# ashual/scene_generation

Measured on AMD Instinct MI355X. Metric: images/sec G+D step, 128x128 <=8-obj scene graphs, higher is better.
Workload: dtype f32

## Files before the change

scene_generation_amd/csrc/common.h:

```cpp
#pragma once
#include <hip/hip_runtime.h>
#include <stdint.h>
#include <stdio.h>
#include <atomic>
#include "../../include/sg2im_hip.h"

#define SG_WAVE 64

void sg_set_error(const char* fmt, ...);
int sg_check_indices_if_enabled(const int64_t* idx, int64_t n, int64_t lo, int64_t hi, const char* what, hipStream_t s);

#define SG_ARG_CHECK(cond, ...)                 \
  do {                                          \
    if (!(cond)) {                              \
      sg_set_error(__VA_ARGS__);                \
      return -1;                                \
    }                                           \
  } while (0)

#define SG_LAUNCH_CHECK(name)                                               \
  do {                                                                      \
    hipError_t e__ = hipGetLastError();                                     \
    if (e__ != hipSuccess) {                                                \
      sg_set_error("%s: launch failed: %s", name, hipGetErrorString(e__)); \
// ... 24 lines not shown
  SG_OPT_BN_BLOCKS,
  SG_OPT_INSTNORM_REG,
  SG_OPT_WGRAD_XCD,
  SG_OPT_WINO_REUSE,
  SG_OPT_WINO_FOLD_CELLS,
  SG_OPT_WINO_PIPE,
  SG_OPT_CHECK_INDICES,
  SG_OPT_LAST_BLOCK,
  SG_OPT_WINO_GEMM_TILE,
  SG_OPT_WINO43,
  SG_OPT_GCONV_FUSED_GATHER,
  SG_OPT_W24_GEMM_TILE,
  SG_OPT_WINO_IN_FUSE,
  SG_OPT_W43_NSUB,
  SG_OPT_W43_KFOLD,
  SG_OPT_WAVE_PRIO,
  SG_OPT_PAR_XCD_CHUNK,
  SG_OPT_W43_TAIL_SPLIT,
  SG_OPT_TAIL_SMAX,
  SG_OPT_TAIL_KTMIN,
  SG_OPT_W43_WGRAD_TILE,
  SG_OPT_PAR_SPLIT,
  SG_OPT_TAIL_CAPTURE,
  SG_OPT_COUNT
};
extern std::atomic<int> g_sg_opt[SG_OPT_COUNT];
static inline int sg_opt(int id) { return g_sg_opt[id].load(std::memory_order_relaxed); }
extern FILE* g_sg_launch_log;

enum {
  SG_K_IGEMM_BASE = 0, SG_K_IGEMM_COUNT = 48,
  SG_K_LINEAR = 48, SG_K_LAYOUT_FWD, SG_K_LAYOUT_BWD, SG_K_INSTNORM, SG_K_BATCHNORM, SG_K_ADAM, SG_K_SEGSUM,
  SG_K_CROP, SG_K_OTHER,
  SG_K_WINO_GEMM_128, SG_K_WINO_GEMM_64, SG_K_WINO_XFORM,
  SG_K_HEAD,
  SG_K_INSTNORM_BWD,
  SG_K_WINO24_GEMM,
  SG_K_WINO43_GEMM,
  SG_K_LAYOUT_TEST_PLANES,
  SG_K_DEPROCESS,
  SG_K_LAYOUT_RGB,
  SG_K_KMEANS_ASSIGN, SG_K_KMEANS_UPDATE, SG_K_KMEANS_RELOCATE, SG_K_KMEANS_PP,
  SG_K_SCENEGRAPH_CENTERS, SG_K_SCENEGRAPH_DERIVE, SG_K_SCENEGRAPH_AGREE,
  SG_K_MAXPOOL3S2, SG_K_ADD_RELU, SG_K_BN_FOLD, SG_K_SGD, SG_K_CLASSIFY_STATS,
  SG_K_RECT_CONV_T64, SG_K_RECT_CONV_T32, SG_K_RECT_CONV_T64W, SG_K_RECT_REDUCE, SG_K_INCEPTION_POOL, SG_K_RESIZE_BILINEAR,
  SG_K_SOFTMAX_ROWS, SG_K_INCEPTION_SCORE,
// ... 93 lines not shown
```

scene_generation_amd/csrc/igemm.hip:

```cpp
#include "igemm_core.h"

namespace sgk {
thread_local double t_alg_bytes = 0.0;
std::mutex g_tab_mu;
std::map<TabKey, TabEntry> g_tabs;
size_t g_tab_bytes = 0;
}

namespace {
int check_desc(const sgConvDesc* d, const char* who) {
  SG_ARG_CHECK(d != nullptr, "%s: null desc", who);
  SG_ARG_CHECK(d->KS == 1 || d->KS == 3 || d->KS == 4 || d->KS == 7, "%s: kernel size %d unsupported", who, d->KS);
  SG_ARG_CHECK(d->stride == 1 || d->stride == 2, "%s: stride %d unsupported", who, d->stride);
  SG_ARG_CHECK(d->upsample == 1 || d->upsample == 2, "%s: upsample %d unsupported", who, d->upsample);
  SG_ARG_CHECK(d->N > 0 && d->C1 > 0 && d->C2 >= 0 && d->Cout > 0 && d->H > 0 && d->W > 0 && d->OH > 0 && d->OW > 0,
               "%s: non-positive dimension", who);
  SG_ARG_CHECK(!d->pad_reflect || d->pad < d->H * d->upsample, "%s: reflect pad too large", who);
  const double lim = SG_MAX_ELEMS;
  SG_ARG_CHECK((double)d->N * (d->C1 + d->C2) * d->H * d->W <= lim && (double)d->N * d->Cout * d->OH * d->OW <= lim &&
                   (double)d->N * (d->C1 + d->C2) * (d->H * d->upsample + 2.0 * d->pad) *
                           (d->W * d->upsample + 2.0 * d->pad) <= lim &&
                   (double)d->Cout * (d->C1 + d->C2) * d->KS * d->KS <= lim,
               "%s: a tensor has more than %.0f elements (32-bit offsets%s)", who, lim,
               SG_BUFLOAD ? ", buffer-load range masking" : "");
// ... 119 lines not shown
extern "C" int sg_conv2d_wgrad(const sgConvDesc* d, const float* gy, const float* x1, const float* x2, float* gw,
                               float* gb, void* ws, size_t ws_bytes, sgStream stream) {
  if (check_desc(d, "sg_conv2d_wgrad")) return -1;
  sgk::t_alg_bytes = 4.0 * ((double)d->N * (d->C1 + d->C2) * d->H * d->W + (double)d->Cout * (d->C1 + d->C2) * d->KS * d->KS + (double)d->N * d->Cout * d->OH * d->OW);
  SG_ARG_CHECK(gy && x1 && gw, "sg_conv2d_wgrad: null pointer");
  SG_ARG_CHECK(d->C2 == 0 || x2, "sg_conv2d_wgrad: C2>0 but x2 null");
  hipStream_t s = (hipStream_t)stream;
  Gather g = make_gather(x1, x2, d->C1, d->C2, d->H, d->W, d->upsample, d->OH, d->OW, d->stride, d->pad, d->pad_reflect);
  g.bcast2 = d->x2_broadcast;
  const double flops = 2.0 * d->Cout * (double)(d->C1 + d->C2) * d->KS * d->KS * d->N * d->OH * d->OW;
  bool gb_done = false;
  if (int rc = sgk::nk_run(d->KS, gy, d->Cout, d->Cout, g, d->N, gw, ws, ws ? ws_bytes : 0, flops, s, nullptr, gb, &gb_done)) return rc;
  SG_LAUNCH_CHECK("sg_conv2d_wgrad");
  if (gb && !gb_done) return sg_channel_sum(gy, gb, d->N, d->Cout, d->OH * d->OW, ws, ws ? ws_bytes : 0, stream);
  return 0;
}


static int check_sparse(const sgConvDesc* d, const int32_t* list, const int32_t* cnt, int L, const char* who) {
  SG_ARG_CHECK(list && cnt, "%s: null channel list", who);
  SG_ARG_CHECK(L > 0 && L <= d->C1 + d->C2, "%s: L=%d outside (0, %d]", who, L, d->C1 + d->C2);
  return 0;
}
extern "C" size_t sg_conv2d_sparse_ws_bytes(const sgConvDesc* d, int L, int kind) {
  if (!d || L <= 0) return 0;
  const int KS2 = d->KS * d->KS;
  if (kind == 0) return sparse_fwd_ws(d->N, d->Cout, L, KS2);
  const size_t a = sparse_wgrad_ws(d->N, d->Cout, d->C1 + d->C2, L, KS2), cs = sg_channel_sum_ws_bytes(d->Cout);
  return a > cs ? a : cs;
}
extern "C" int sg_conv2d_fwd_sparse(const sgConvDesc* d, const float* x1, const float* x2, const float* w,
                                    const float* bias, const int32_t* chan_list, const int32_t* chan_cnt, int L, float* y,
                                    int act, float slope, void* ws, size_t ws_bytes, sgStream stream) {
  if (check_desc(d, "sg_conv2d_fwd_sparse") || check_sparse(d, chan_list, chan_cnt, L, "sg_conv2d_fwd_sparse")) return -1;
  sgk::t_alg_bytes = 4.0 * ((double)d->N * L * d->H * d->W + (double)d->N * d->Cout * L * d->KS * d->KS + (double)d->N * d->Cout * d->OH * d->OW);
  SG_ARG_CHECK(x1 && w && y && ws, "sg_conv2d_fwd_sparse: null pointer");
  SG_ARG_CHECK(d->C2 == 0 || x2, "sg_conv2d_fwd_sparse: C2>0 but x2 null");
  SG_ARG_CHECK(ws_bytes >= sg_conv2d_sparse_ws_bytes(d, L, 0), "sg_conv2d_fwd_sparse: workspace too small");
  hipStream_t s = (hipStream_t)stream;
  const int K = (d->C1 + d->C2) * d->KS * d->KS;
  Gather g = make_gather(x1, x2, d->C1, d->C2, d->H, d->W, d->upsample, d->OH, d->OW, d->stride, d->pad, d->pad_reflect);
  g.bcast2 = d->x2_broadcast;
  const Sparse sp{chan_list, chan_cnt, L, nullptr, nullptr};
  int rc = sgk::kn_sparse_run(d->KS, w, d->Cout, K, g, d->N, bias, y, act, slope, sp, ws, s);
  SG_LAUNCH_CHECK("sg_conv2d_fwd_sparse");
  return rc;
}
extern "C" int sg_conv2d_wgrad_sparse(const sgConvDesc* d, const float* gy, const float* x1, const float* x2,
                                      const int32_t* chan_list, const int32_t* chan_cnt, int L, float* gw, float* gb,
                                      void* ws, size_t ws_bytes, sgStream stream) {
  if (check_desc(d, "sg_conv2d_wgrad_sparse") || check_sparse(d, chan_list, chan_cnt, L, "sg_conv2d_wgrad_sparse")) return -1;
  sgk::t_alg_bytes = 4.0 * ((double)d->N * L * d->H * d->W + (double)d->N * d->Cout * L * d->KS * d->KS + (double)d->N * d->Cout * d->OH * d->OW);
  SG_ARG_CHECK(gy && x1 && gw && ws, "sg_conv2d_wgrad_sparse: null pointer");
  SG_ARG_CHECK(d->C2 == 0 || x2, "sg_conv2d_wgrad_sparse: C2>0 but x2 null");
  SG_ARG_CHECK(ws_bytes >= sg_conv2d_sparse_ws_bytes(d, L, 2), "sg_conv2d_wgrad_sparse: workspace too small");
  hipStream_t s = (hipStream_t)stream;
  Gather g = make_gather(x1, x2, d->C1, d->C2, d->H, d->W, d->upsample, d->OH, d->OW, d->stride, d->pad, d->pad_reflect);
  g.bcast2 = d->x2_broadcast;
  const Sparse sp{chan_list, chan_cnt, L, nullptr, nullptr};
  if (int rc = sgk::nk_run(d->KS, gy, d->Cout, d->Cout, g, d->N, gw, ws, ws_bytes, 0.0, s, &sp)) return rc;
  SG_LAUNCH_CHECK("sg_conv2d_wgrad_sparse");
  if (gb) return sg_channel_sum(gy, gb, d->N, d->Cout, d->OH * d->OW, ws, ws_bytes, stream);
  return 0;
}
extern "C" int sg_conv2d_fwd_perimage(const sgConvDesc* d, const float* x1, const float* x2, const float* wimg,
                                      const float* bias, const int32_t* chan_list, const int32_t* chan_cnt, int L, float* y,
                                      int act, float slope, void* ws, size_t ws_bytes, sgStream stream) {
  if (check_desc(d, "sg_conv2d_fwd_perimage") || check_sparse(d, chan_list, chan_cnt, L, "sg_conv2d_fwd_perimage")) return -1;
  sgk::t_alg_bytes = 4.0 * ((double)d->N * L * d->H * d->W + (double)d->N * d->Cout * L * d->KS * d->KS + (double)d->N * d->Cout * d->OH * d->OW);
  SG_ARG_CHECK(x1 && wimg && y && ws, "sg_conv2d_fwd_perimage: null pointer");
  SG_ARG_CHECK(d->C2 == 0 || x2, "sg_conv2d_fwd_perimage: C2>0 but x2 null");
  SG_ARG_CHECK(ws_bytes >= sg_conv2d_sparse_ws_bytes(d, L, 0), "sg_conv2d_fwd_perimage: workspace too small");
  hipStream_t s = (hipStream_t)stream;
  const int K = (d->C1 + d->C2) * d->KS * d->KS;
  Gather g = make_gather(x1, x2, d->C1, d->C2, d->H, d->W, d->upsample, d->OH, d->OW, d->stride, d->pad, d->pad_reflect);
  g.bcast2 = d->x2_broadcast;
  const Sparse sp{chan_list, chan_cnt, L, wimg, nullptr};
  int rc = sgk::kn_sparse_run(d->KS, nullptr, d->Cout, K, g, d->N, bias, y, act, slope, sp, ws, s);
  SG_LAUNCH_CHECK("sg_conv2d_fwd_perimage");
  return rc;
}
extern "C" int sg_conv2d_wgrad_perimage(const sgConvDesc* d, const float* gy, const float* x1, const float* x2,
                                        const int32_t* chan_list, const int32_t* chan_cnt, int L, float* gwimg, void* ws,
                                        size_t ws_bytes, sgStream stream) {
  if (check_desc(d, "sg_conv2d_wgrad_perimage") || check_sparse(d, chan_list, chan_cnt, L, "sg_conv2d_wgrad_perimage")) return -1;
  sgk::t_alg_bytes = 4.0 * ((double)d->N * L * d->H * d->W + (double)d->N * d->Cout * L * d->KS * d->KS + (double)d->N * d->Cout * d->OH * d->OW);
  SG_ARG_CHECK(gy && x1 && gwimg && ws, "sg_conv2d_wgrad_perimage: null pointer");
  SG_ARG_CHECK(d->C2 == 0 || x2, "sg_conv2d_wgrad_perimage: C2>0 but x2 null");
  SG_ARG_CHECK(ws_bytes >= sg_conv2d_sparse_ws_bytes(d, L, 2), "sg_conv2d_wgrad_perimage: workspace too small");
  hipStream_t s = (hipStream_t)stream;
  Gather g = make_gather(x1, x2, d->C1, d->C2, d->H, d->W, d->upsample, d->OH, d->OW, d->stride, d->pad, d->pad_reflect);
  g.bcast2 = d->x2_broadcast;
  const Sparse sp{chan_list, chan_cnt, L, nullptr, gwimg};
  if (int rc = sgk::nk_run(d->KS, gy, d->Cout, d->Cout, g, d->N, nullptr, ws, ws_bytes, 0.0, s, &sp)) return rc;
  SG_LAUNCH_CHECK("sg_conv2d_wgrad_perimage");
  return 0;
}

extern "C" int sg_convT2d_fwd(const sgConvDesc* d, const float* x, const float* w, const float* bias, float* y,
                              void* ws, size_t ws_bytes, sgStream stream) {
  if (check_desc(d, "sg_convT2d_fwd")) return -1;
  sgk::t_alg_bytes = 4.0 * ((double)d->N * (d->C1) * d->H * d->W + (double)d->Cout * (d->C1) * d->KS * d->KS + (double)d->N * d->Cout * d->OH * d->OW);
  SG_ARG_CHECK(x && w && y && ws, "sg_convT2d_fwd: null pointer");
  const int Cin = d->C1, R = d->KS * d->KS;
  SG_ARG_CHECK(d->C2 == 0 && d->upsample == 1 && !d->pad_reflect, "sg_convT2d_fwd: unsupported desc");
  SG_ARG_CHECK(ws_bytes >= (size_t)d->Cout * Cin * R * sizeof(float) + ktab_bytes(Cin * R),
               "sg_convT2d_fwd: workspace too small");
  hipStream_t s = (hipStream_t)stream;
  const TgArgs ta = tg_args(d, SG_TG_CONVT_FWD, 0, 0);
  Gather g = make_gather(x, nullptr, Cin, 0, d->H, d->W, 1, ta.PH, ta.PW, d->stride, ta.pad, 0);
  const double flops = 2.0 * d->Cout * Cin * R * (double)d->N * d->H * d->W;
  if (ta.parity) {
    SG_ARG_CHECK(ws_bytes >= parity_ws(d->Cout, Cin, R), "sg_convT2d_fwd: workspace too small");
    int rc = sgk::kn_parity_run(d->KS, w, Cin, d->Cout, 0, ta.M, g, d->N, bias, y, d->Cout, SG_ACT_NONE, 0.f, flops, ws,
                              ws_bytes, s);
    SG_LAUNCH_CHECK("sg_convT2d_fwd");
// ... 2130 lines not shown
```

scene_generation_amd/csrc/igemm_core.h:

```cpp
#pragma once
#include <type_traits>
#include "common.h"
#include <stdlib.h>
#include <array>
#include <map>
#include <mutex>

typedef float f32x16 __attribute__((ext_vector_type(16)));


namespace sgk {
struct Gather {
  const float* src1; const float* src2;
  int C1, C2;
  int SH, SW;
  int LH, LW;
  int ushift;
  int PH, PW;
  int stride, sshift, pad, reflect;
  int bcast2;
  int pstep, ph0, pw0;
};

struct KEntry { unsigned choff; unsigned tapsel; };
struct Sparse { const int* list; const int* cnt; int L; const float* wimg; float* gwimg; };
struct TabEntry { void* dev; size_t bytes; hipEvent_t ready; hipStream_t stream; };
using TabKey = std::array<long long, 12>;
extern thread_local double t_alg_bytes;
extern std::mutex g_tab_mu;
extern std::map<TabKey, TabEntry> g_tabs;
extern size_t g_tab_bytes;

int kn0_run(int KS, const float* A, int M, int K, const Gather& g, int NB, const float* bias, float* out, int Mtot, int act,
            float slope, double flops, void* ktab_ws, size_t ws_avail, hipStream_t s);
int kn1_run(int KS, const float* A, int M, int K, const Gather& g, int NB, const float* bias, float* out, int Mtot, int act,
            float slope, double flops, void* ktab_ws, size_t ws_avail, unsigned variant_stride, hipStream_t s);
int kn_sparse_run(int KS, const float* W, int M, int K, const Gather& g, int NB, const float* bias, float* out, int act,
                  float slope, const Sparse& sp, void* ws, hipStream_t s);
int kn_parity_run(int KS, const float* W, int Rdim, int B, int m0, int M, const Gather& g, int NB, const float* bias,
                  float* out, int Mtot, int act, float slope, double flops, void* ws, size_t ws_bytes, hipStream_t s);
int nk_run(int KS, const float* A, int M, int Mtot, const Gather& g, int NB, float* out, void* ws, size_t ws_bytes,
           double flops, hipStream_t s, const Sparse* sp, float* gb = nullptr, bool* gb_done = nullptr);
int skinny_vec(int align, int ld, int K);
int skinny_gemm(const float* a, int lda, int av, const float* b, int ldb, int bv, float* c, const float* bias,
                float* rowsum, int M, int N, int K, int act, float slope, hipStream_t s);
int skinny_gemm_gather(const float* obj, const float* pred, const int64_t* edges, int T, int Do, int Dp, const float* w, float* c,
                       const float* bias, int N, int act, float slope, hipStream_t s);
inline bool skinny_shape(int M, int N) {
// ... 730 lines not shown
#endif
    const bool ok = !MASK || o1 >= 0;
    const unsigned b1 = ok ? (unsigned)o1 : 0u;
    const unsigned b2 = (TWO && ok) ? (unsigned)buf[2 * KBLK + kl_] : 0u;
#pragma unroll
    for (int j = 0; j < COLS; ++j) {
      if (TWO) {
        const bool second = (secmask_ >> j) & 1u;
        const float* base = second ? g.src2 : g.src1;
        st.r[j] = base[(second ? b2 : b1) + choff_[j]];
      } else {
        st.r[j] = g.src1[b1 + choff_[j]];
      }
    }
    st.ok = ok ? 1u : 0u;
  }
  __device__ __forceinline__ void store(const Stage& st, float* T) const {
    const bool ok = !MASK || st.ok != 0u;
#pragma unroll
    for (int j = 0; j < COLS; ++j) T[(nr_ + 16 * j) * LDK + kl_] = ok ? st.r[j] : 0.f;
  }
};

template <int ACT> __device__ __forceinline__ float act_fixed(float v, int act, float slope) {
  if constexpr (ACT == SG_ACT_NONE) return v;
  else if constexpr (ACT == SG_ACT_RELU) return v > 0.f ? v : 0.f;
  else if constexpr (ACT == SG_ACT_LEAKY) return v > 0.f ? v : v * slope;
  else return sg_apply_act(v, act, slope);
}
template <int A> struct ActTag { static constexpr int value = A; };
template <class F> __device__ __forceinline__ void ep_dispatch(bool full, int act, F&& f) {
  if (full && act == SG_ACT_NONE) f(ActTag<SG_ACT_NONE>{});
  else if (full && act == SG_ACT_LEAKY) f(ActTag<SG_ACT_LEAKY>{});
  else if (full && act == SG_ACT_RELU) f(ActTag<SG_ACT_RELU>{});
  else f(ActTag<-1>{});
}

struct EpNCHW {
  float* out; const float* bias; int PHW, Mtot, M, Npix, act; float slope; size_t zstride;
  int PWs, step, h0, w0, PWf, PHWf;
  FastDiv dPHW, dPWs;
  __device__ __forceinline__ void set_limit(int n) { Npix = n; }
  template <int TM, int TN>
  __device__ __forceinline__ void store(f32x16 (&acc)[TM][TN], int mbase, int nbase, int lane, int z) const {
    const bool full = mbase + 32 * TM <= M && nbase + 32 * TN <= Npix;
    const int mrow = mbase + 4 * (lane >> 5);
// ... 963 lines not shown
  } else {
    t.Rdim = d->Cout; t.M = c_end - c_begin; t.PH = d->H; t.PW = d->W; t.pad = 1;
  }
  t.K = t.Rdim * R;
  t.a_off = t.parity ? 0 : (entry == SG_TG_CONVT_FWD ? 0 : (size_t)c_begin * t.K);
  t.ws_off = t.parity ? 0 : nw * sizeof(float);
  if (entry == SG_TG_DGRAD_FOLDED) {
    const size_t VS = (size_t)d->N * d->Cout * d->OH * d->OW;
    t.variants = (unsigned)VS;
    t.ws_off = (((nw + 63) / 64) * 64 + 9 * VS) * sizeof(float);
  }
  return t;
}

inline int sparse_kc(int L, int KS2) { return sg_cdiv(L * KS2, BK) * BK; }
inline int sparse_kpad(int L, int KS2) { return sg_cdiv(sparse_kc(L, KS2), 64) * 64 + 128; }
inline size_t sparse_fwd_ws(int NB, int M, int L, int KS2) {
  return (size_t)NB * ((size_t)sparse_kpad(L, KS2) * sizeof(KEntry) + (size_t)M * sparse_kc(L, KS2) * sizeof(float) + 64);
}
inline size_t parity_ws(int M, int Rdim, int KS2) { return (size_t)M * Rdim * KS2 * sizeof(float) + 64; }
inline size_t sparse_wgrad_ws(int NB, int M, int C, int L, int KS2) {
  return (size_t)NB * M * (sg_cdiv(L, 128) * 128) * KS2 * sizeof(float) + (size_t)NB * C * sizeof(int);
}
struct NkPlan { int tile; bool tap; int cpad; int splits; };
inline NkPlan nk_plan(int M, int C, int KS2, int Kpix, bool two) {
  NkPlan p;
  p.tap = C >= 48 || two;
  p.tile = M <= 32 ? 2 : 1;
  if (M > 64 && p.tap) {
    const double w128 = (double)sg_cdiv(M, 128) * 128 * sg_cdiv(C, 128) * 128;
    const double w64 = (double)sg_cdiv(M, 64) * 64 * sg_cdiv(C, 64) * 64;
    if (w128 * 0.7 < w64) p.tile = 0;
  }
  const int BMt = p.tile == 0 ? 128 : ((p.tile == 1 || p.tile == 3) ? 64 : 32), BNt = p.tile == 1 ? 64 : 128;
  p.cpad = p.tap ? sg_cdiv(C, BNt) * BNt : 0;
  const long tiles = (long)sg_cdiv(M, BMt) * (p.tap ? (long)KS2 * (p.cpad / BNt) : (long)sg_cdiv((long)C * KS2, BNt));
  const int target = p.tile == 0 ? 768 : 1024;
  int s = (int)((target + tiles - 1) / tiles);
  const int maxs = Kpix / (BK * 8) > 0 ? Kpix / (BK * 8) : 1;
  if (s > maxs) s = maxs;
  const int cap = p.tap ? 64 : 256;
  if (s > cap) s = cap;
  if (sg_opt(SG_OPT_WGRAD_XCD) && s >= 6) {
    int s8 = (s + 7) / 8 * 8;
    if (s8 > maxs) s8 = maxs / 8 * 8;
    if (s8 >= 8) s = s8;
// ... 7 lines not shown
```

scene_generation_amd/csrc/igemm_nk.hip:

```cpp
#include "igemm_core.h"

namespace {
__global__ void sparse_inv_kernel(const int* list, const int* cnt, int L, int C, int* inv) {
  const int b = blockIdx.y, c = blockIdx.x * blockDim.x + threadIdx.x;
  if (c >= C) return;
  int pos = -1;
  const int n = cnt[b];
  for (int j = 0; j < n; ++j) pos = list[b * L + j] == c ? j : pos;
  inv[b * C + c] = pos;
}
__global__ void sparse_wgrad_reduce_kernel(const float* slabs, const int* inv, float* gw, int M, int C, int KS2, int cpad,
                                           int NB) {
  const size_t i = (size_t)blockIdx.x * blockDim.x + threadIdx.x;
  if (i >= (size_t)M * C * KS2) return;
  const int t = (int)(i % KS2);
  const int c = (int)((i / KS2) % C);
  const int m = (int)(i / ((size_t)KS2 * C));
  float v = 0.f;
  for (int b = 0; b < NB; ++b) {
    const int j = inv[b * C + c];
    if (j >= 0) v += slabs[(((size_t)b * M + m) * KS2 + t) * cpad + j];
  }
  gw[i] = v;
}
// ... 9 lines not shown
                                             int NB) {
  const size_t i = (size_t)blockIdx.x * blockDim.x + threadIdx.x;
  if (i >= (size_t)NB * M * L * KS2) return;
  const int t = (int)(i % KS2);
  const int j = (int)((i / KS2) % L);
  const size_t bm = i / ((size_t)KS2 * L);
  const int b = (int)(bm / M);
  gwimg[i] = j < cnt[b] ? slabs[(bm * KS2 + t) * cpad + j] : 0.f;
}
__global__ void wgrad_unpermute_reduce_kernel(const float* __restrict__ slabs, float* __restrict__ gw, int M, int C, int KS2,
                                              int cpad, int S, const float* __restrict__ rowsum, float* __restrict__ gb) {
  const unsigned j = blockIdx.x * blockDim.x + threadIdx.x;
  const int m = blockIdx.y;
  if (gb && j == 0) {
    const float b = sg_sum_strided(rowsum + m, (size_t)M, S);
    gb[m] = b;
  }
  if (j >= (unsigned)(C * KS2)) return;
  const unsigned c = j / (unsigned)KS2, t = j - c * (unsigned)KS2;
  const size_t zs = (size_t)M * KS2 * cpad;
  const float* p = slabs + ((size_t)m * KS2 + t) * cpad + c;
  const float v = sg_sum_strided(p, zs, S);
  gw[(size_t)m * C * KS2 + j] = v;
}
template <int KS>
void launch_nk_general(int tile, const float* A, int M, int Mtot, int PQ, const Gather& g, int Ncols, const EpRowMajor& ep,
                       int Kpix, int splits, hipStream_t s, const Sparse* sp = nullptr, int zdiv = 1) {
  float* const rowsum = nullptr;
  const FastDiv dPQ((unsigned)PQ);
  const int* sl = sp ? sp->list : nullptr; const int* sc = sp ? sp->cnt : nullptr; const int L = sp ? sp->L : 0;
  if (tile == 2)
    launch_cfg<CfgW32>(LoadPixK<32>{A, M, Mtot, PQ, dPQ, rowsum}, LoadGatherNK<128, KS, false, true, NSW>{g, Ncols, sl, sc, L, zdiv}, ep,
                       M, Ncols, Kpix, splits, s);
  else if (KS == 7 && sp && (PQ % 4 == 0) && aligned16(A))
    launch_cfg<CfgW64>(LoadPixKVec<64>{A, M, Mtot, PQ, dPQ, rowsum}, LoadGatherNK<64, KS, false, true, NSW>{g, Ncols, sl, sc, L, zdiv}, ep,
                       M, Ncols, Kpix, splits, s);
  else
    launch_cfg<CfgW64>(LoadPixK<64>{A, M, Mtot, PQ, dPQ, rowsum}, LoadGatherNK<64, KS, false, true, NSW>{g, Ncols, sl, sc, L, zdiv}, ep,
                       M, Ncols, Kpix, splits, s);
}

template <class CFG, int BMv, int BNv>
void launch_nk_tap(const float* A, int M, int Mtot, int PQ, bool vecA, const Gather& g, int KS, int Ccols, int cpad,
                   const Sparse* sp, bool nomask, const EpWgrad& ep, int Kpix, int splits, hipStream_t s, float* rowsum) {
  const FastDiv dPQ((unsigned)PQ), dPW((unsigned)g.PW);
  const int* sl = sp ? sp->list : nullptr; const int* sc = sp ? sp->cnt : nullptr; const int L = sp ? sp->L : 0;
// ... 19 lines not shown
  if (gb_done) *gb_done = false;
  const int PQ = g.PH * g.PW, KS2 = KS * KS;
  const int Kpix = NB * PQ;
  const int C = g.C1 + g.C2;
  const int Ccols = sp ? sp->L : C;
  const int Ncols = Ccols * KS2;
  NkPlan pl = nk_plan(M, Ccols, KS2, Kpix, g.C2 > 0);
  if (sp && sp->gwimg && g.C2 == 0 && sg_cdiv(Ccols, 64) * 64 >= 3 * Ccols) {
    const int tile = M <= 32 ? 2 : 1;
    const long tiles = (long)sg_cdiv(M, tile == 2 ? 32 : 64) * sg_cdiv(Ncols, tile == 2 ? 128 : 64) * NB;
    int S = (int)((1024 + tiles - 1) / tiles);
    if (S > 128 / Ccols) S = 128 / Ccols;
    if (S > PQ / 256) S = PQ / 256;
    if (S < 1) S = 1;
    const int kcs = sg_cdiv(sg_cdiv(PQ, S), BK) * BK;
    S = sg_cdiv(PQ, kcs);
    const size_t mnc = (size_t)M * Ncols;
    SG_ARG_CHECK(ws && ws_bytes >= mnc * sizeof(float) * (size_t)S * NB, "wgrad: workspace too small");
    float* dstp = S > 1 ? reinterpret_cast<float*>(ws) : sp->gwimg;
    const EpRowMajor ep{dstp, nullptr, M, Ncols, Ncols, SG_ACT_NONE, 0.f, mnc};
    t_batch = BatchInfo{}; t_batch.kimg = PQ; t_batch.ksplit = S; t_batch.kcs = kcs;
    t_grid_z = NB * S;
    t_xcd_z = sg_opt(SG_OPT_WGRAD_XCD) ? 2 : 0;
    {
      SgProfScope prof(sg_igemm_kind(2, KS, tile), s, 2.0 * M * (double)Ncols * Kpix, 0);
      switch (KS) {
        case 1: launch_nk_general<1>(tile, A, M, Mtot, PQ, g, Ncols, ep, Kpix, 1, s, sp, S); break;
        case 3: launch_nk_general<3>(tile, A, M, Mtot, PQ, g, Ncols, ep, Kpix, 1, s, sp, S); break;
        case 4: launch_nk_general<4>(tile, A, M, Mtot, PQ, g, Ncols, ep, Kpix, 1, s, sp, S); break;
        case 7: launch_nk_general<7>(tile, A, M, Mtot, PQ, g, Ncols, ep, Kpix, 1, s, sp, S); break;
      }
    }
    t_batch = BatchInfo{};
    t_grid_z = 0;
    t_xcd_z = 0;
    if (S > 1)
      hipLaunchKernelGGL(slab_group_reduce_kernel, dim3(sg_cdiv(mnc * NB, 256)), dim3(256), 0, s, (const float*)ws, sp->gwimg,
                         mnc, S, NB);
    return 0;
  }
  if (sp) pl.tap = true;
  if (sp && pl.cpad == 0) pl.cpad = sg_cdiv(Ccols, pl.tile == 1 ? 64 : 128) * (pl.tile == 1 ? 64 : 128);
  int splits = sp ? NB : pl.splits;
  const size_t mn = pl.tap ? (size_t)M * KS2 * pl.cpad : (size_t)M * Ncols;
  if (!sp && splits > 1 && ws_bytes < mn * sizeof(float) * (size_t)splits) splits = (int)(ws_bytes / (mn * sizeof(float)));
  if (!sp && splits < 2) splits = 1;
  SG_ARG_CHECK(!pl.tap || (ws && ws_bytes >= mn * sizeof(float) * (size_t)splits), "wgrad: workspace too small");
// ... 85 lines not shown
```

scene_generation_amd/csrc/norm.hip:

```cpp
#include "common.h"
#include <stdlib.h>

namespace {

__device__ __forceinline__ float act_grad_from_pre(float pre, int act, float slope) {
  switch (act) {
    case SG_ACT_RELU: return pre > 0.f ? 1.f : 0.f;
    case SG_ACT_LEAKY: return pre > 0.f ? 1.f : slope;
    default: return 1.f;
  }
}

template <bool WAVE>
__global__ void __launch_bounds__(256) instnorm_fwd_kernel(const float* __restrict__ x, const float* __restrict__ skip,
                                                          float* __restrict__ y, float* __restrict__ mean_o,
                                                          float* __restrict__ rstd_o, int NC, int HW, float eps, int act,
                                                          float slope) {
  __shared__ float red[16];
  const int lane = threadIdx.x & 63;
  const int plane = WAVE ? blockIdx.x * 4 + (threadIdx.x >> 6) : blockIdx.x;
  if (WAVE && plane >= NC) return;
  const int t0 = WAVE ? lane : threadIdx.x, nt = WAVE ? 64 : blockDim.x;
  const float* xp = x + (size_t)plane * HW;
  float s = 0.f;
// ... 967 lines not shown
}

__global__ void pad_upsample_bwd_kernel(const float* __restrict__ gp, float* __restrict__ gx, int H, int W, int pad, int ups) {
  const unsigned j = blockIdx.x * blockDim.x + threadIdx.x;
  if (j >= (unsigned)(H * W)) return;
  const size_t nc = blockIdx.y;
  const int h = (int)(j / (unsigned)W), w = (int)(j - (unsigned)h * (unsigned)W);
  const int LH = H * ups, LW = W * ups, PH = LH + 2 * pad, PW = LW + 2 * pad;
  const float* g = gp + nc * PH * PW;
  float s = 0.f;
  for (int dh = 0; dh < ups; ++dh) {
    int ah[3];
    const int nh = reflect_sources(h * ups + dh, LH, pad, ah);
    for (int dw = 0; dw < ups; ++dw) {
      int aw[3];
      const int nw = reflect_sources(w * ups + dw, LW, pad, aw);
      for (int a = 0; a < nh; ++a)
        for (int b = 0; b < nw; ++b) s += g[ah[a] * PW + aw[b]];
    }
  }
  gx[nc * H * W + j] = s;
}

__global__ void concat_channels_kernel(const float* __restrict__ a, const float* __restrict__ b, float* __restrict__ out,
                                       size_t total, int Ca, int Cb, int HW) {
  const size_t i = (size_t)blockIdx.x * blockDim.x + threadIdx.x;
  if (i >= total) return;
  const int p = i % HW;
  const int c = (i / HW) % (Ca + Cb);
  const size_t n = i / ((size_t)HW * (Ca + Cb));
  out[i] = c < Ca ? a[(n * Ca + c) * HW + p] : b[(n * Cb + (c - Ca)) * HW + p];
}


__global__ void pool2d_fwd_kernel(const float* __restrict__ x, float* __restrict__ y, size_t total, int H, int W, int OH,
                                  int OW, int k, int avg) {
  const size_t i = (size_t)blockIdx.x * blockDim.x + threadIdx.x;
  if (i >= total) return;
  const int ow = i % OW;
  const int oh = (i / OW) % OH;
  const size_t nc = i / ((size_t)OW * OH);
  const float* p = x + (nc * H + (size_t)oh * k) * W + (size_t)ow * k;
  float m = p[0], s = 0.f;
  for (int a = 0; a < k; ++a)
    for (int b = 0; b < k; ++b) {
      const float v = p[(size_t)a * W + b];
// ... 377 lines not shown
extern "C" int sg_replicate_pad_fwd(const float* x, float* y, int NC, int H, int W, int pad, sgStream stream) {
  SG_ARG_CHECK(x && y && NC > 0 && H > 0 && W > 0 && pad >= 0, "sg_replicate_pad_fwd: bad arguments");
  const size_t total = (size_t)NC * (H + 2 * pad) * (W + 2 * pad);
  hipLaunchKernelGGL(replicate_pad_fwd_kernel, grid1d(total), dim3(256), 0, (hipStream_t)stream, x, y, total, H, W, pad);
  SG_LAUNCH_CHECK("sg_replicate_pad_fwd");
  return 0;
}

extern "C" int sg_replicate_pad_bwd(const float* gp, float* gx, int NC, int H, int W, int pad, sgStream stream) {
  SG_ARG_CHECK(gp && gx && NC > 0 && H > 0 && W > 0 && pad >= 0, "sg_replicate_pad_bwd: bad arguments");
  const size_t total = (size_t)NC * H * W;
  hipLaunchKernelGGL(replicate_pad_bwd_kernel, grid1d(total), dim3(256), 0, (hipStream_t)stream, gp, gx, total, H, W, pad);
  SG_LAUNCH_CHECK("sg_replicate_pad_bwd");
  return 0;
}

extern "C" int sg_pad_upsample_bwd(const float* gp, float* gx, int NC, int H, int W, int pad, int upsample,
                                   sgStream stream) {
  SG_ARG_CHECK(gp && gx && (upsample == 1 || upsample == 2) && pad >= 0, "sg_pad_upsample_bwd: bad arguments");
  if (NC == 0 || H * W == 0) return 0;
  for (int n0 = 0; n0 < NC; n0 += 65535) {
    const int nn = NC - n0 < 65535 ? NC - n0 : 65535;
    const size_t PP = (size_t)(H * upsample + 2 * pad) * (W * upsample + 2 * pad);
    hipLaunchKernelGGL(pad_upsample_bwd_kernel, dim3(sg_cdiv(H * W, 256), nn), dim3(256), 0, (hipStream_t)stream,
                       gp + (size_t)n0 * PP, gx + (size_t)n0 * H * W, H, W, pad, upsample);
  }
  SG_LAUNCH_CHECK("sg_pad_upsample_bwd");
  return 0;
}

extern "C" int sg_concat_channels(const float* a, const float* b, float* out, int N, int Ca, int Cb, int HW,
                                  sgStream stream) {
  SG_ARG_CHECK(a && b && out, "sg_concat_channels: bad arguments");
  const size_t total = (size_t)N * (Ca + Cb) * HW;
  hipLaunchKernelGGL(concat_channels_kernel, grid1d(total), dim3(256), 0, (hipStream_t)stream, a, b, out, total, Ca, Cb, HW);
  SG_LAUNCH_CHECK("sg_concat_channels");
  return 0;
}

extern "C" int sg_cond_conv_split_w(const float* w, float* w1, float* w2r, int M, int C1, int C2, int R, sgStream stream) {
  SG_ARG_CHECK(w && w1 && w2r && M > 0 && C1 > 0 && C2 > 0 && R > 0, "sg_cond_conv_split_w: bad arguments");
  const size_t total = (size_t)M * (C1 + C2) * R;
  hipLaunchKernelGGL(cond_split_w_kernel, grid1d(total), dim3(256), 0, (hipStream_t)stream, w, w1, w2r, total, C1, C2, R);
  SG_LAUNCH_CHECK("sg_cond_conv_split_w");
  return 0;
}
// ... 35 lines not shown
```

scene_generation_amd/csrc/runtime.hip:

```cpp
#include "common.h"
#include <stdarg.h>
#include <mutex>
#include <vector>
#include <stdlib.h>
#include <string.h>
#include <ctype.h>

static thread_local char t_err[512] = "ok";

void sg_set_error(const char* fmt, ...) {
  va_list ap;
  va_start(ap, fmt);
  vsnprintf(t_err, sizeof(t_err), fmt, ap);
  va_end(ap);
}

extern "C" const char* sg_last_error_string(void) { return t_err; }
extern "C" int sg_version(void) { return 100; }

int g_sg_prof_on = 0;

std::atomic<int> g_sg_opt[SG_OPT_COUNT];
FILE* g_sg_launch_log = nullptr;
namespace {
struct OptDef { const char* name; int def; };
const OptDef kOpts[SG_OPT_COUNT] = {
    {"tile", -1}, {"t128_min", 384}, {"tile3", 1}, {"tile3_min", 768}, {"split_target", 1536}, {"split_kmin", 2048}, {"splits", -1}, {"fixedtap", 1}, {"wino_wt", 1},
    {"w24_small", 1}, {"w24_s", -1}, {"w24_pmin", 256}, {"wino_adjoint", 1}, {"wino24", 1}, {"linear_nsub", 2},
    {"linear_skinny", 2048}, {"wgrad_rowsum", 1}, {"layout_reg", 1}, {"layout_dsplit", 1}, {"bn_blocks", 4096},
    {"instnorm_reg", 2}, {"wgrad_xcd", 1}, {"wino_reuse", 1}, {"wino_fold_cells", 1}, {"wino_pipe", 2},
    {"check_indices", 0}, {"last_block", 0}, {"wino_gemm_tile", 0}, {"wino43", 1}, {"gconv_fused_gather", 1}, {"w24_gemm_tile", 2}, {"wino_in_fuse", 1}, {"w43_nsub", 1}, {"w43_kfold", 256}, {"wave_prio", 0}, {"par_xcd_chunk", 16}, {"w43_tail_split", 2}, {"tail_smax", 4}, {"tail_ktmin", 8}, {"w43_wgrad_tile", 0}, {"par_split", 1}, {"tail_capture", 1}};
struct OptInit {
  OptInit() {
    for (int i = 0; i < SG_OPT_COUNT; ++i) {
      char env[64] = "SG_";
      size_t n = 3;
      for (const char* c = kOpts[i].name; *c && n + 1 < sizeof(env); ++c) env[n++] = (char)toupper((unsigned char)*c);
      env[n] = 0;
      const char* e = getenv(env);
      g_sg_opt[i].store((e && *e) ? atoi(e) : kOpts[i].def, std::memory_order_relaxed);
    }
    const char* lf = getenv("SG_LAUNCH_LOG");
    if (lf && *lf) g_sg_launch_log = fopen(lf, "a");
  }
} g_opt_init;
int opt_index(const char* key) {
  if (!key) return -1;
  for (int i = 0; i < SG_OPT_COUNT; ++i)
    if (strcmp(key, kOpts[i].name) == 0) return i;
  return -1;
}
}

extern "C" int sg_num_options(void) { return SG_OPT_COUNT; }
// ... 177 lines not shown
```

Baseline: 1122.

## Pre-pad reflect planes for 7x7 sparse wgrad and vectorize reflect-pad backward fold

For 7x7 stride-1 reflect-padded per-image sparse weight gradients, a new kernel first materializes reflect-padded copies of the selected input channel planes in extra workspace. The GEMM then loads from them with buffer loads using precomputed column offsets, replacing per-element reflect and bounds gather logic. Separately, the pad backward for upsample==1 now copies the interior with float4 and only sums the 3x3 reflected contributions on the border ring. The trade-offs are extra workspace and an extra padding pass per call.

Measured after the change: 1136 (median of 6 runs). 1.3% higher.

```diff
diff --git a/scene_generation_amd/csrc/common.h b/scene_generation_amd/csrc/common.h
--- a/scene_generation_amd/csrc/common.h
+++ b/scene_generation_amd/csrc/common.h
@@ -70,6 +70,7 @@
   SG_OPT_W43_WGRAD_TILE,
   SG_OPT_PAR_SPLIT,
   SG_OPT_TAIL_CAPTURE,
+  SG_OPT_WGRAD_PADDED,
   SG_OPT_COUNT
 };
 extern std::atomic<int> g_sg_opt[SG_OPT_COUNT];
diff --git a/scene_generation_amd/csrc/igemm.hip b/scene_generation_amd/csrc/igemm.hip
--- a/scene_generation_amd/csrc/igemm.hip
+++ b/scene_generation_amd/csrc/igemm.hip
@@ -165,12 +165,19 @@
   SG_ARG_CHECK(L > 0 && L <= d->C1 + d->C2, "%s: L=%d outside (0, %d]", who, L, d->C1 + d->C2);
   return 0;
 }
+static size_t sparse_wgrad_base_ws(const sgConvDesc* d, int L) {
+  const size_t a = sparse_wgrad_ws(d->N, d->Cout, d->C1 + d->C2, L, d->KS * d->KS), cs = sg_channel_sum_ws_bytes(d->Cout);
+  return a > cs ? a : cs;
+}
+static size_t sparse_wgrad_padded_bytes(const sgConvDesc* d, int L) {
+  return nk_padded_bytes(d->KS, d->N, L, d->C2, d->H, d->W, d->upsample, d->OH, d->OW, d->stride, d->pad, d->pad_reflect);
+}
 extern "C" size_t sg_conv2d_sparse_ws_bytes(const sgConvDesc* d, int L, int kind) {
   if (!d || L <= 0) return 0;
   const int KS2 = d->KS * d->KS;
   if (kind == 0) return sparse_fwd_ws(d->N, d->Cout, L, KS2);
-  const size_t a = sparse_wgrad_ws(d->N, d->Cout, d->C1 + d->C2, L, KS2), cs = sg_channel_sum_ws_bytes(d->Cout);
-  return a > cs ? a : cs;
+  const size_t base = sparse_wgrad_base_ws(d, L), pb = sparse_wgrad_padded_bytes(d, L);
+  return pb ? nk_padded_offset(base) + pb : base;
 }
 extern "C" int sg_conv2d_fwd_sparse(const sgConvDesc* d, const float* x1, const float* x2, const float* w,
                                     const float* bias, const int32_t* chan_list, const int32_t* chan_cnt, int L, float* y,
@@ -196,7 +203,7 @@
   sgk::t_alg_bytes = 4.0 * ((double)d->N * L * d->H * d->W + (double)d->N * d->Cout * L * d->KS * d->KS + (double)d->N * d->Cout * d->OH * d->OW);
   SG_ARG_CHECK(gy && x1 && gw && ws, "sg_conv2d_wgrad_sparse: null pointer");
   SG_ARG_CHECK(d->C2 == 0 || x2, "sg_conv2d_wgrad_sparse: C2>0 but x2 null");
-  SG_ARG_CHECK(ws_bytes >= sg_conv2d_sparse_ws_bytes(d, L, 2), "sg_conv2d_wgrad_sparse: workspace too small");
+  SG_ARG_CHECK(ws_bytes >= sparse_wgrad_base_ws(d, L), "sg_conv2d_wgrad_sparse: workspace too small");
   hipStream_t s = (hipStream_t)stream;
   Gather g = make_gather(x1, x2, d->C1, d->C2, d->H, d->W, d->upsample, d->OH, d->OW, d->stride, d->pad, d->pad_reflect);
   g.bcast2 = d->x2_broadcast;
@@ -230,11 +237,13 @@
   sgk::t_alg_bytes = 4.0 * ((double)d->N * L * d->H * d->W + (double)d->N * d->Cout * L * d->KS * d->KS + (double)d->N * d->Cout * d->OH * d->OW);
   SG_ARG_CHECK(gy && x1 && gwimg && ws, "sg_conv2d_wgrad_perimage: null pointer");
   SG_ARG_CHECK(d->C2 == 0 || x2, "sg_conv2d_wgrad_perimage: C2>0 but x2 null");
-  SG_ARG_CHECK(ws_bytes >= sg_conv2d_sparse_ws_bytes(d, L, 2), "sg_conv2d_wgrad_perimage: workspace too small");
+  const size_t base = sparse_wgrad_base_ws(d, L), pb = sparse_wgrad_padded_bytes(d, L);
+  SG_ARG_CHECK(ws_bytes >= base, "sg_conv2d_wgrad_perimage: workspace too small");
   hipStream_t s = (hipStream_t)stream;
   Gather g = make_gather(x1, x2, d->C1, d->C2, d->H, d->W, d->upsample, d->OH, d->OW, d->stride, d->pad, d->pad_reflect);
   g.bcast2 = d->x2_broadcast;
-  const Sparse sp{chan_list, chan_cnt, L, nullptr, gwimg};
+  Sparse sp{chan_list, chan_cnt, L, nullptr, gwimg};
+  if (pb && ws_bytes >= nk_padded_offset(base) + pb) sp.pad_off = nk_padded_offset(base);
   if (int rc = sgk::nk_run(d->KS, gy, d->Cout, d->Cout, g, d->N, nullptr, ws, ws_bytes, 0.0, s, &sp)) return rc;
   SG_LAUNCH_CHECK("sg_conv2d_wgrad_perimage");
   return 0;
diff --git a/scene_generation_amd/csrc/igemm_core.h b/scene_generation_amd/csrc/igemm_core.h
--- a/scene_generation_amd/csrc/igemm_core.h
+++ b/scene_generation_amd/csrc/igemm_core.h
@@ -23,7 +23,7 @@
 };
 
 struct KEntry { unsigned choff; unsigned tapsel; };
-struct Sparse { const int* list; const int* cnt; int L; const float* wimg; float* gwimg; };
+struct Sparse { const int* list; const int* cnt; int L; const float* wimg; float* gwimg; size_t pad_off = 0; };
 struct TabEntry { void* dev; size_t bytes; hipEvent_t ready; hipStream_t stream; };
 using TabKey = std::array<long long, 12>;
 extern thread_local double t_alg_bytes;
@@ -800,6 +800,56 @@
   }
 };
 
+constexpr unsigned PAD_INVALID = 1u << 28;
+constexpr size_t PAD_MAX_BYTES = (size_t)1 << 30;
+template <int BN, int KS, int NS = SG_NSUB>
+struct LoadPaddedNK {
+  const float* pp; unsigned bytes;
+  int PQ, PW, PWp, PP, L;
+  const int* chan_cnt;
+  FastDiv dPQ, dPW;
+  static constexpr int KS2 = KS * KS;
+  static constexpr int LDS_INTS = 2 * KBLK;
+  static constexpr int COLS = BN / 16;
+  struct Stage { float r[COLS]; };
+  int kl_, tid_, nr_, kbeg_, kend_;
+  unsigned coloff_[COLS];
+  int* lds_;
+  __device__ __forceinline__ void set_batch(int, int, int) {}
+  __device__ __forceinline__ void init(int n0, int tid, int* lds, int kbeg, int kend) {
+    kl_ = tid & 15; nr_ = tid >> 4; tid_ = tid; lds_ = lds; kbeg_ = kbeg; kend_ = kend;
+    const int ncols = chan_cnt[kbeg / PQ] * KS2;
+#pragma unroll
+    for (int j = 0; j < COLS; ++j) {
+      const int n = n0 + nr_ + 16 * j;
+      const int cj = n / KS2, t = n - cj * KS2;
+      const int kh = t / KS, kw = t - kh * KS;
+      coloff_[j] = n < ncols ? (unsigned)(cj * PP + kh * PWp + kw) : PAD_INVALID;
+    }
+  }
+  __device__ __forceinline__ void prefetch(Stage&, int k0) const {
+    const int rel = k0 - kbeg_;
+    if ((rel & (KBLK - 1)) != 0) return;
+    const int k = k0 + tid_;
+    const unsigned kk = k < kend_ ? (unsigned)k : 0u;
+    const unsigned img = dPQ.div(kk), pix = kk - img * (unsigned)PQ;
+    const unsigned ph = dPW.div(pix), pw = pix - ph * (unsigned)PW;
+    lds_[((rel / KBLK) & 1) * KBLK + tid_] = k < kend_ ? (int)(img * (unsigned)(L * PP) + ph * (unsigned)PWp + pw) : (int)PAD_INVALID;
+  }
+  __device__ __forceinline__ void load(Stage& st, int k0, int) const {
+    const int rel = k0 - kbeg_;
+    const unsigned p0 = (unsigned)lds_[((rel / KBLK) & 1) * KBLK + (rel & (KBLK - 1)) + kl_];
+    const __amdgpu_buffer_rsrc_t r = __builtin_amdgcn_make_buffer_rsrc(const_cast<float*>(pp), 0, bytes, 0x00020000);
+#pragma unroll
+    for (int j = 0; j < COLS; ++j)
+      st.r[j] = __builtin_bit_cast(float, __builtin_amdgcn_raw_buffer_load_b32(r, (int)((p0 + coloff_[j]) << 2), 0, 0));
+  }
+  __device__ __forceinline__ void store(const Stage& st, float* T) const {
+#pragma unroll
+    for (int j = 0; j < COLS; ++j) T[(nr_ + 16 * j) * LDK + kl_] = st.r[j];
+  }
+};
+
 template <int ACT> __device__ __forceinline__ float act_fixed(float v, int act, float slope) {
   if constexpr (ACT == SG_ACT_NONE) return v;
   else if constexpr (ACT == SG_ACT_RELU) return v > 0.f ? v : 0.f;
@@ -1809,6 +1859,13 @@
 inline size_t sparse_wgrad_ws(int NB, int M, int C, int L, int KS2) {
   return (size_t)NB * M * (sg_cdiv(L, 128) * 128) * KS2 * sizeof(float) + (size_t)NB * C * sizeof(int);
 }
+inline size_t nk_padded_bytes(int KS, int NB, int L, int C2, int SH, int SW, int ups, int PH, int PW, int stride, int pad, int reflect) {
+  if (!(KS == 7 && reflect && C2 == 0 && ups == 1 && stride == 1 && pad >= 1 && pad < SH && pad < SW && NB > 0 && L > 0)) return 0;
+  if (PH != SH + 2 * pad - KS + 1 || PW != SW + 2 * pad - KS + 1 || PH < 1 || PW < 1) return 0;
+  const size_t b = (size_t)NB * L * (SH + 2 * pad) * (SW + 2 * pad) * sizeof(float);
+  return b <= PAD_MAX_BYTES ? b : 0;
+}
+inline size_t nk_padded_offset(size_t base_bytes) { return (base_bytes + 255) / 256 * 256; }
 struct NkPlan { int tile; bool tap; int cpad; int splits; };
 inline NkPlan nk_plan(int M, int C, int KS2, int Kpix, bool two) {
   NkPlan p;
diff --git a/scene_generation_amd/csrc/igemm_nk.hip b/scene_generation_amd/csrc/igemm_nk.hip
--- a/scene_generation_amd/csrc/igemm_nk.hip
+++ b/scene_generation_amd/csrc/igemm_nk.hip
@@ -55,6 +55,34 @@
   const float* p = slabs + ((size_t)m * KS2 + t) * cpad + c;
   const float v = sg_sum_strided(p, zs, S);
   gw[(size_t)m * C * KS2 + j] = v;
+}
+__global__ void reflect_pad_planes_kernel(const float* __restrict__ x, const int* __restrict__ list, const int* __restrict__ cnt,
+                                          float* __restrict__ pp, int C, int L, int H, int W, int pad, int PWp, int PP,
+                                          FastDiv dPWp) {
+  const unsigned e = blockIdx.x * blockDim.x + threadIdx.x;
+  const int j = blockIdx.y, b = blockIdx.z;
+  if (e >= (unsigned)PP || j >= cnt[b]) return;
+  const unsigned oh = dPWp.div(e), ow = e - oh * (unsigned)PWp;
+  int ih = (int)oh - pad, iw = (int)ow - pad;
+  ih = ih < 0 ? -ih : (ih >= H ? 2 * H - 2 - ih : ih);
+  iw = iw < 0 ? -iw : (iw >= W ? 2 * W - 2 - iw : iw);
+  const int c = list[b * L + j];
+  pp[((size_t)b * L + j) * PP + e] = x[((size_t)b * C + c) * ((size_t)H * W) + (unsigned)(ih * W + iw)];
+}
+void launch_nk_padded(int tile, const float* A, int M, int Mtot, int PQ, const Gather& g, int Ncols, const EpRowMajor& ep, int Kpix,
+                      hipStream_t s, const Sparse& sp, const float* pp) {
+  float* const rowsum = nullptr;
+  const FastDiv dPQ((unsigned)PQ), dPW((unsigned)g.PW);
+  const int PWp = g.SW + 2 * g.pad, PP = (g.SH + 2 * g.pad) * PWp;
+  const unsigned bytes = (unsigned)((size_t)(Kpix / PQ) * sp.L * PP * sizeof(float));
+#define SG_PAD_B(BNv) LoadPaddedNK<BNv, 7, NSW>{pp, bytes, PQ, g.PW, PWp, PP, sp.L, sp.cnt, dPQ, dPW}
+  if (tile == 2)
+    launch_cfg<CfgW32>(LoadPixK<32>{A, M, Mtot, PQ, dPQ, rowsum}, SG_PAD_B(128), ep, M, Ncols, Kpix, 1, s);
+  else if ((PQ % 4 == 0) && aligned16(A))
+    launch_cfg<CfgW64>(LoadPixKVec<64>{A, M, Mtot, PQ, dPQ, rowsum}, SG_PAD_B(64), ep, M, Ncols, Kpix, 1, s);
+  else
+    launch_cfg<CfgW64>(LoadPixK<64>{A, M, Mtot, PQ, dPQ, rowsum}, SG_PAD_B(64), ep, M, Ncols, Kpix, 1, s);
+#undef SG_PAD_B
 }
 template <int KS>
 void launch_nk_general(int tile, const float* A, int M, int Mtot, int PQ, const Gather& g, int Ncols, const EpRowMajor& ep,
@@ -120,7 +148,17 @@
     t_batch = BatchInfo{}; t_batch.kimg = PQ; t_batch.ksplit = S; t_batch.kcs = kcs;
     t_grid_z = NB * S;
     t_xcd_z = sg_opt(SG_OPT_WGRAD_XCD) ? 2 : 0;
-    {
+    const size_t pbytes = nk_padded_bytes(KS, NB, Ccols, g.C2, g.SH, g.SW, g.ushift ? 2 : 1, g.PH, g.PW, g.stride, g.pad, g.reflect);
+    const bool padded = sg_opt(SG_OPT_WGRAD_PADDED) && pbytes > 0 && sp->pad_off >= mnc * sizeof(float) * (size_t)S * NB &&
+                        g.pstep == 1 && NB <= 65535 && ws_bytes >= sp->pad_off + pbytes;
+    if (padded) {
+      float* pp = reinterpret_cast<float*>(reinterpret_cast<char*>(ws) + sp->pad_off);
+      const int PWp = g.SW + 2 * g.pad, PP = (g.SH + 2 * g.pad) * PWp;
+      hipLaunchKernelGGL(reflect_pad_planes_kernel, dim3(sg_cdiv(PP, 256), Ccols, NB), dim3(256), 0, s, g.src1, sp->list, sp->cnt, pp,
+                         g.C1, Ccols, g.SH, g.SW, g.pad, PWp, PP, FastDiv((unsigned)PWp));
+      SgProfScope prof(sg_igemm_kind(2, KS, tile), s, 2.0 * M * (double)Ncols * Kpix, 0);
+      launch_nk_padded(tile, A, M, Mtot, PQ, g, Ncols, ep, Kpix, s, *sp, pp);
+    } else {
       SgProfScope prof(sg_igemm_kind(2, KS, tile), s, 2.0 * M * (double)Ncols * Kpix, 0);
       switch (KS) {
         case 1: launch_nk_general<1>(tile, A, M, Mtot, PQ, g, Ncols, ep, Kpix, 1, s, sp, S); break;
diff --git a/scene_generation_amd/csrc/norm.hip b/scene_generation_amd/csrc/norm.hip
--- a/scene_generation_amd/csrc/norm.hip
+++ b/scene_generation_amd/csrc/norm.hip
@@ -1013,6 +1013,67 @@
   gx[nc * H * W + j] = s;
 }
 
+struct FoldPlan {
+  int hq0, hq1, wq0, wq1, iblocks;
+  FastDiv dnq, dW, dWb;
+};
+__global__ void __launch_bounds__(256) reflect_fold_kernel(const float* __restrict__ gp, float* __restrict__ gx, int H, int W,
+                                                           int pad, FoldPlan fp) {
+  const size_t nc = blockIdx.y;
+  const int PW = W + 2 * pad, PH = H + 2 * pad;
+  const float* g = gp + nc * PH * PW;
+  float* o = gx + nc * H * W;
+  const int rows = fp.hq1 - fp.hq0, nq = (fp.wq1 - fp.wq0) >> 2;
+  if ((int)blockIdx.x < fp.iblocks) {
+    const unsigned id = blockIdx.x * 256u + threadIdx.x;
+    if (id >= (unsigned)(rows * nq)) return;
+    const unsigned r = fp.dnq.div(id), q = id - r * (unsigned)nq;
+    const int h = fp.hq0 + (int)r, w0 = fp.wq0 + 4 * (int)q;
+    const float* src = g + (unsigned)((h + pad) * PW + pad + w0);
+    float* dst = o + (unsigned)(h * W + w0);
+    float4 v;
+    if ((reinterpret_cast<uintptr_t>(src) & 15) == 0) v = *reinterpret_cast<const float4*>(src);
+    else v = make_float4(src[0], src[1], src[2], src[3]);
+    v = make_float4(0.f + v.x, 0.f + v.y, 0.f + v.z, 0.f + v.w);
+    if ((reinterpret_cast<uintptr_t>(dst) & 15) == 0) *reinterpret_cast<float4*>(dst) = v;
+    else { dst[0] = v.x; dst[1] = v.y; dst[2] = v.z; dst[3] = v.w; }
+    return;
+  }
+  const unsigned id = (blockIdx.x - (unsigned)fp.iblocks) * 256u + threadIdx.x;
+  const int Wb = W - 4 * nq, ntb = (H - rows) * W;
+  if (id >= (unsigned)(ntb + rows * Wb)) return;
+  int h, w;
+  if (id < (unsigned)ntb) {
+    const unsigned r = fp.dW.div(id);
+    w = (int)(id - r * (unsigned)W);
+    h = (int)r < fp.hq0 ? (int)r : (int)r - fp.hq0 + fp.hq1;
+  } else {
+    const unsigned e = id - (unsigned)ntb, r = fp.dWb.div(e);
+    const int c = (int)(e - r * (unsigned)Wb);
+    h = fp.hq0 + (int)r;
+    w = c < fp.wq0 ? c : c - fp.wq0 + fp.wq1;
+  }
+  const int ih[3] = {h + pad, pad - h, pad + 2 * H - 2 - h};
+  const bool lh[3] = {true, h >= 1 && h <= pad, h <= H - 2 && h >= H - 1 - pad};
+  const int iw[3] = {w + pad, pad - w, pad + 2 * W - 2 - w};
+  const bool lw[3] = {true, w >= 1 && w <= pad, w <= W - 2 && w >= W - 1 - pad};
+  float v[3][3];
+#pragma unroll
+  for (int a = 0; a < 3; ++a)
+#pragma unroll
+    for (int b = 0; b < 3; ++b) {
+      const bool live = lh[a] && lw[b];
+      v[a][b] = g[live ? ih[a] * PW + iw[b] : ih[0] * PW + iw[0]];
+      v[a][b] = live ? v[a][b] : 0.f;
+    }
+  float s = 0.f;
+#pragma unroll
+  for (int a = 0; a < 3; ++a)
+#pragma unroll
+    for (int b = 0; b < 3; ++b) s += v[a][b];
+  o[h * W + w] = s;
+}
+
 __global__ void concat_channels_kernel(const float* __restrict__ a, const float* __restrict__ b, float* __restrict__ out,
                                        size_t total, int Ca, int Cb, int HW) {
   const size_t i = (size_t)blockIdx.x * blockDim.x + threadIdx.x;
@@ -1436,6 +1497,18 @@
   for (int n0 = 0; n0 < NC; n0 += 65535) {
     const int nn = NC - n0 < 65535 ? NC - n0 : 65535;
     const size_t PP = (size_t)(H * upsample + 2 * pad) * (W * upsample + 2 * pad);
+    if (upsample == 1) {
+      FoldPlan fp;
+      fp.hq0 = pad + 1; fp.hq1 = H - 1 - pad; fp.wq0 = (pad + 1 + 3) & ~3; fp.wq1 = (W - 1 - pad) & ~3;
+      if (fp.hq1 <= fp.hq0 || fp.wq1 <= fp.wq0) { fp.hq0 = fp.hq1 = 0; fp.wq0 = fp.wq1 = 0; }
+      const int rows = fp.hq1 - fp.hq0, nq = (fp.wq1 - fp.wq0) / 4, Wb = W - 4 * nq;
+      fp.iblocks = sg_cdiv(rows * nq, 256);
+      fp.dnq = FastDiv((unsigned)(nq > 0 ? nq : 1)); fp.dW = FastDiv((unsigned)W); fp.dWb = FastDiv((unsigned)(Wb > 0 ? Wb : 1));
+      const int ring = (H - rows) * W + rows * Wb;
+      hipLaunchKernelGGL(reflect_fold_kernel, dim3(fp.iblocks + sg_cdiv(ring, 256), nn), dim3(256), 0, (hipStream_t)stream,
+                         gp + (size_t)n0 * PP, gx + (size_t)n0 * H * W, H, W, pad, fp);
+      continue;
+    }
     hipLaunchKernelGGL(pad_upsample_bwd_kernel, dim3(sg_cdiv(H * W, 256), nn), dim3(256), 0, (hipStream_t)stream,
                        gp + (size_t)n0 * PP, gx + (size_t)n0 * H * W, H, W, pad, upsample);
   }
diff --git a/scene_generation_amd/csrc/runtime.hip b/scene_generation_amd/csrc/runtime.hip
--- a/scene_generation_amd/csrc/runtime.hip
+++ b/scene_generation_amd/csrc/runtime.hip
@@ -29,7 +29,7 @@
     {"w24_small", 1}, {"w24_s", -1}, {"w24_pmin", 256}, {"wino_adjoint", 1}, {"wino24", 1}, {"linear_nsub", 2},
     {"linear_skinny", 2048}, {"wgrad_rowsum", 1}, {"layout_reg", 1}, {"layout_dsplit", 1}, {"bn_blocks", 4096},
     {"instnorm_reg", 2}, {"wgrad_xcd", 1}, {"wino_reuse", 1}, {"wino_fold_cells", 1}, {"wino_pipe", 2},
-    {"check_indices", 0}, {"last_block", 0}, {"wino_gemm_tile", 0}, {"wino43", 1}, {"gconv_fused_gather", 1}, {"w24_gemm_tile", 2}, {"wino_in_fuse", 1}, {"w43_nsub", 1}, {"w43_kfold", 256}, {"wave_prio", 0}, {"par_xcd_chunk", 16}, {"w43_tail_split", 2}, {"tail_smax", 4}, {"tail_ktmin", 8}, {"w43_wgrad_tile", 0}, {"par_split", 1}, {"tail_capture", 1}};
+    {"check_indices", 0}, {"last_block", 0}, {"wino_gemm_tile", 0}, {"wino43", 1}, {"gconv_fused_gather", 1}, {"w24_gemm_tile", 2}, {"wino_in_fuse", 1}, {"w43_nsub", 1}, {"w43_kfold", 256}, {"wave_prio", 0}, {"par_xcd_chunk", 16}, {"w43_tail_split", 2}, {"tail_smax", 4}, {"tail_ktmin", 8}, {"w43_wgrad_tile", 0}, {"par_split", 1}, {"tail_capture", 1}, {"wgrad_padded", 1}};
 struct OptInit {
   OptInit() {
     for (int i = 0; i < SG_OPT_COUNT; ++i) {
```
